# WeltXing/PyDyNet

Hardware: AMD Instinct MI355X
Metric: training-step samples/sec (6L Llama3, seq=256) (higher is better)
Workload: dtype f32

## Files before the change

pydynet_amd/csrc/common.h:

```cpp
#pragma once
#include <hip/hip_runtime.h>
#include <stdint.h>
#include <stdio.h>
#include <string.h>

#define PDN_MAX_DIMS 8

enum {
  PDN_OK = 0,
  PDN_EINVAL = -1,
  PDN_EUNSUPPORTED = -2,
  PDN_EWORKSPACE = -3,
};

void pdn_set_error(const char* fmt, ...);

enum {
  PDN_CNT_ROWRES_CHUNK = 0,
  PDN_CNT_ROWTILE_PLAIN = 1,
  PDN_CNT_ROWTILE_SWIGLU_FWD = 2,
  PDN_CNT_ROWTILE_SWIGLU_BWD = 3,
  PDN_CNT_ROWTILE_ROPE = 4,
  PDN_CNT_ROWTILE_ROWMAX = 5,
  PDN_CNT_ROWRES_CHUNK_EPI = 6,
  PDN_CNT_ATT_P_FWD = 7,
  PDN_CNT_ATT_P_BWD = 8,
  PDN_CNT_ATT_RES_FWD = 9,
  PDN_CNT_ATT_RES_BWD = 10,
  PDN_CNT_ATT_STREAM = 11,
  PDN_CNT_CE_DX_DEFERRED = 12,
  PDN_CNT_CE_DW = 13,
  PDN_CNT_OUTRES = 14,
  PDN_CNT_OUTRES_TN = 15,
  PDN_CNT_LINEAR_RELU_FWD = 16,
  PDN_CNT_LINEAR_DX_MASKED = 17,
  PDN_CNT_CE_SMALL = 18,
  PDN_CNT_TILED_SWIGLU_FWD = 19,
  PDN_CNT_TILED_SWIGLU_BWD = 20,
  PDN_CNT_CONV_QUAD_FWD = 21,
  PDN_CNT_CONV_QUAD_DGRAD = 22,
  PDN_CNT_CONV_QUAD_WGRAD = 23,
  PDN_CNT_PATCH_EMBED_FWD = 24,
  PDN_CNT_PATCH_EMBED_BWD = 25,
  PDN_CNT_L2NORM_FWD = 26,
  PDN_CNT_L2NORM_BWD = 27,
  PDN_CNT_SAMPLE = 28,
  PDN_CNT_DECODE_ROWS = 29,
  PDN_CNT_DECODE_SLOTS = 30,
  PDN_CNT_DECODE_WIDE = 31,
  PDN_CNT_BEAM = 32,
  PDN_CNT_EXTEND = 33,
  PDN_CNT_SPECULATE = 34,
  PDN_CNT_PENALTY = 35,
  PDN_CNT_LOGPROBS = 36,
  PDN_CNT_LMHEAD_SPLIT = 37,
  PDN_CNT_PREFIX = 38,
  PDN_CNT_CE_DX_SPLIT = 39,
  PDN_CNT_CE_DW_SPLIT = 40,
  PDN_CNT_ROWTILE_SPLIT = 41,
  PDN_CNT_OUTRES_TN_SPLIT = 42,
  PDN_CNT_ATT_SEG = 43,
  PDN_CNT_ROW_LOSS = 44,
  PDN_CNT_SMOOTH_LOSS = 45,
  PDN_CNT_SLOTS = 46
};
void pdn_count(int slot);

#define PDN_CHECK_ARG(cond, ...)          \
  do {                                    \
    if (!(cond)) {                        \
      pdn_set_error(__VA_ARGS__);         \
      return PDN_EINVAL;                  \
    }                                     \
  } while (0)

#define PDN_LAUNCH_CHECK()                                            \
  do {                                                                \
    hipError_t _e = hipGetLastError();                                \
    if (_e != hipSuccess) {                                           \
      pdn_set_error("%s:%d launch failed: %s", __FILE__, __LINE__,    \
                    hipGetErrorString(_e));                           \
      return (int)_e;                                                 \
    }                                                                 \
  } while (0)

#define PDN_HIP(call)                                                 \
  do {                                                                \
    hipError_t _e = (call);                                           \
    if (_e != hipSuccess) {                                           \
      pdn_set_error("%s:%d %s: %s", __FILE__, __LINE__, #call,        \
                    hipGetErrorString(_e));                           \
      return (int)_e;                                                 \
    }                                                                 \
  } while (0)

static inline int64_t cdiv64(int64_t a, int64_t b) { return (a + b - 1) / b; }

struct PdnView {
  int ndim;
  int64_t shape[PDN_MAX_DIMS];
  int64_t stride[PDN_MAX_DIMS];
};

__device__ __forceinline__ float wave_sum(float v) {
#pragma unroll
  for (int o = 32; o > 0; o >>= 1) v += __shfl_xor(v, o, 64);
  return v;
}
__device__ __forceinline__ float wave_max(float v) {
#pragma unroll
  for (int o = 32; o > 0; o >>= 1) v = fmaxf(v, __shfl_xor(v, o, 64));
  return v;
}
__device__ __forceinline__ double wave_sum(double v) {
#pragma unroll
  for (int o = 32; o > 0; o >>= 1) v += __shfl_xor(v, o, 64);
  return v;
}

template <typename T>
__device__ __forceinline__ T block_sum(T v, T* smem) {
  v = wave_sum(v);
  const int lane = threadIdx.x & 63, wid = threadIdx.x >> 6, nw = (blockDim.x + 63) >> 6;
  if (nw == 1) return v;
  __syncthreads();
  if (lane == 0) smem[wid] = v;
  __syncthreads();
  T r = (T)0;
  for (int i = 0; i < nw; ++i) r += smem[i];
  return r;
}
__device__ __forceinline__ void lds_barrier() {
  asm volatile("s_waitcnt lgkmcnt(0)" ::: "memory");
  __builtin_amdgcn_s_barrier();
  asm volatile("" ::: "memory");
}
__device__ __forceinline__ float block_sum_lds(float v, float* smem) {
  v = wave_sum(v);
  const int lane = threadIdx.x & 63, wid = threadIdx.x >> 6, nw = (blockDim.x + 63) >> 6;
  if (nw == 1) return v;
  lds_barrier();
  if (lane == 0) smem[wid] = v;
  lds_barrier();
  float r = 0.f;
  for (int i = 0; i < nw; ++i) r += smem[i];
  return r;
}
__device__ __forceinline__ float block_max_lds(float v, float* smem) {
  v = wave_max(v);
  const int lane = threadIdx.x & 63, wid = threadIdx.x >> 6, nw = (blockDim.x + 63) >> 6;
  if (nw == 1) return v;
  lds_barrier();
  if (lane == 0) smem[wid] = v;
  lds_barrier();
  float r = smem[0];
  for (int i = 1; i < nw; ++i) r = fmaxf(r, smem[i]);
  return r;
}
__device__ __forceinline__ float block_max(float v, float* smem) {
  v = wave_max(v);
  const int lane = threadIdx.x & 63, wid = threadIdx.x >> 6, nw = (blockDim.x + 63) >> 6;
  if (nw == 1) return v;
  __syncthreads();
  if (lane == 0) smem[wid] = v;
  __syncthreads();
  float r = smem[0];
  for (int i = 1; i < nw; ++i) r = fmaxf(r, smem[i]);
  return r;
}
```

pydynet_amd/csrc/gemm_outres.hip:

```cpp
#include "common.h"
#include <stdlib.h>

static int pdn_ablation_switch(const char* name) {
  const char* e = getenv(name);
  const int v = e ? atoi(e) : 0;
  if (v) fprintf(stderr, "[pdnhip] WARNING: %s=%d -- timing ablation active, results of the affected kernels are WRONG\n", name, v);
  return v;
}

typedef float f32x16 __attribute__((ext_vector_type(16)));

struct OutResParams {
  const float* A;
  const float* B;
  float* C;
  const float* bias;
  const float* residual;
  int M, K;
  int64_t lda, ldb, ldc;
  const float* lse;
  const int64_t* targets;
  const float* gdev;
  float gscale;
  int kps;
// ... 92 lines not shown
      const int I = min(q * NW + wave, 35);
      *reinterpret_cast<float4*>(smem + buf * PIECE + I * 256 + 4 * lane) = rb[q];
    }
  };

  if (npieces > s0) {
#pragma unroll
    for (int q = 0; q < NQ; ++q) issue_one(0, s0, q);
    if (STAGE) park(0);
  }
  const int arow_i = min(m0 + li, p.M - 1);
  const float* arow = p.A + (int64_t)arow_i * p.lda + 4 * lh;
  float4 a[4];
#pragma unroll
  for (int g = 0; g < 4; ++g) {
    const float4 v = *reinterpret_cast<const float4*>(arow + (int64_t)s0 * OR_KP + 8 * g);
    a[g].x = v.x; a[g].y = v.y; a[g].z = v.z; a[g].w = v.w;
  }
  float ce_lse = 0.f, ce_sc = 0.f;
  int ce_rel = 0;
  if (CE == 1) {
    ce_lse = p.lse[arow_i];
    ce_rel = (int)p.targets[arow_i] - 4 * lh;
    ce_sc = p.gscale * (p.gdev ? p.gdev[0] : 1.f);
  }
  float ce_c2 = 0.f, ce_z = 0.f;
  float ce_m = 0.f;
  if (CE == 2) {
    ce_m = p.lse[arow_i];
    for (int q = 1; q < p.max_parts; ++q) ce_m = fmaxf(ce_m, p.lse[(int64_t)q * p.M + arow_i]);
    ce_c2 = -ce_m * 1.4426950408889634f;
  }

  f32x16 acc[9];
#pragma unroll
  for (int j = 0; j < 9; ++j)
#pragma unroll
    for (int r = 0; r < 16; ++r) acc[j][r] = 0.f;

  const int xl = (li >> 1) & 7;
  const int bnn = (4 * lh) * OR_N + li;
  int bq[4];
#pragma unroll
  for (int g = 0; g < 4; ++g) bq[g] = BT ? li * OR_KP + 4 * ((2 * g + lh) ^ xl) : 0;

  for (int s = s0; s < npieces; ++s) {
    if (STAGE) asm volatile("s_waitcnt lgkmcnt(0)" ::: "memory");
    else if (s == s0) asm volatile("s_waitcnt vmcnt(0)" ::: "memory");
    else asm volatile("s_waitcnt vmcnt(2)" ::: "memory");
    __builtin_amdgcn_s_barrier();
    asm volatile("" ::: "memory");
    const float* Bp = smem + ((s - s0) & 1) * PIECE;
    const int nxt = min(s + 1, npieces - 1);
    const float* anext = arow + (int64_t)nxt * OR_KP;
    float b0[3][4], b1[3][4];
#define OR_LOADB(BX, G, T)                                                                       \
  if (BT) {                                                                                      \
    _Pragma("unroll") for (int j = 0; j < 3; ++j) {                                              \
      const float4 v = *reinterpret_cast<const float4*>(Bp + bq[G] + (3 * (T) + j) * (32 * OR_KP)); \
      BX[j][0] = v.x; BX[j][1] = v.y; BX[j][2] = v.z; BX[j][3] = v.w;                            \
    }                                                                                            \
  } else {                                                                                       \
    _Pragma("unroll") for (int j = 0; j < 3; ++j)                                                \
      _Pragma("unroll") for (int q = 0; q < 4; ++q) BX[j][q] = Bp[bnn + (8 * (G) + q) * OR_N + 32 * (3 * (T) + j)]; \
  }
#define OR_MFMA(BX, AV, T)                                                                       \
  {                                                                                              \
    _Pragma("unroll") for (int j = 0; j < 3; ++j) acc[3 * (T) + j] = __builtin_amdgcn_mfma_f32_32x32x2f32(AV.x, BX[j][0], acc[3 * (T) + j], 0, 0, 0); \
    _Pragma("unroll") for (int j = 0; j < 3; ++j) acc[3 * (T) + j] = __builtin_amdgcn_mfma_f32_32x32x2f32(AV.y, BX[j][1], acc[3 * (T) + j], 0, 0, 0); \
    _Pragma("unroll") for (int j = 0; j < 3; ++j) acc[3 * (T) + j] = __builtin_amdgcn_mfma_f32_32x32x2f32(AV.z, BX[j][2], acc[3 * (T) + j], 0, 0, 0); \
    _Pragma("unroll") for (int j = 0; j < 3; ++j) acc[3 * (T) + j] = __builtin_amdgcn_mfma_f32_32x32x2f32(AV.w, BX[j][3], acc[3 * (T) + j], 0, 0, 0); \
  }
#define OR_STEP(BC, BN, G, T)                                                                    \
  if (3 * (G) + (T) + 1 < 12) { OR_LOADB(BN, (3 * (G) + (T) + 1) / 3, (3 * (G) + (T) + 1) % 3) }  \
  __builtin_amdgcn_sched_barrier(0);                                                             \
  OR_MFMA(BC, av, T)                                                                             \
  __builtin_amdgcn_sched_barrier(0);
    OR_LOADB(b0, 0, 0)
#pragma unroll
    for (int g = 0; g < 4; ++g) {
      float4 av = a[g];
      if (CE == 1) {
        const int c0 = ce_rel - (OR_KP * s + 8 * g);
        av.x = ce_grad(av.x, ce_lse, c0 == 0, ce_sc); av.y = ce_grad(av.y, ce_lse, c0 == 1, ce_sc);
        av.z = ce_grad(av.z, ce_lse, c0 == 2, ce_sc); av.w = ce_grad(av.w, ce_lse, c0 == 3, ce_sc);
      }
      if (CE == 2) {
        const float L2E = 1.4426950408889634f;
        av.x = __builtin_amdgcn_exp2f(fmaf(av.x, L2E, ce_c2)); av.y = __builtin_amdgcn_exp2f(fmaf(av.y, L2E, ce_c2));
        av.z = __builtin_amdgcn_exp2f(fmaf(av.z, L2E, ce_c2)); av.w = __builtin_amdgcn_exp2f(fmaf(av.w, L2E, ce_c2));
        ce_z += (av.x + av.y) + (av.z + av.w);
      }
      if (g < 3 && (!(ABLATE & 2) || s < 1)) {
#pragma unroll
        for (int e = 0; e < 3; ++e)
          if (3 * g + e < NQ) issue_one((s - s0 + 1) & 1, nxt, 3 * g + e);
      }
      __builtin_amdgcn_sched_barrier(0);
      if (g & 1) {
        OR_STEP(b1, b0, g, 0) OR_STEP(b0, b1, g, 1) OR_STEP(b1, b0, g, 2)
      } else {
        OR_STEP(b0, b1, g, 0) OR_STEP(b1, b0, g, 1) OR_STEP(b0, b1, g, 2)
      }
      if (!(ABLATE & 1)) {
        const float4 v = *reinterpret_cast<const float4*>(anext + 8 * g);
        a[g].x = v.x; a[g].y = v.y; a[g].z = v.z; a[g].w = v.w;
      }
      __builtin_amdgcn_sched_barrier(0);
    }
#undef OR_STEP
    if (STAGE) park((s - s0 + 1) & 1);
#undef OR_LOADB
#undef OR_MFMA
  }
  asm volatile("s_waitcnt vmcnt(0)" ::: "memory");

  if (CE == 2 && p.slab) {
    const float z = ce_z + __shfl_xor(ce_z, 32, 64);
    if (lh == 0 && m0 + li < p.M) p.zslab[(int64_t)blockIdx.y * p.M + m0 + li] = z;
  }
  if (CE == 2 && !p.slab) {
    const float z = ce_z + __shfl_xor(ce_z, 32, 64);
    const float izl = 1.f / z;
    const int tgl = min(max((int)p.targets[arow_i], 0), p.K - 1);
    if (lh == 0 && m0 + li < p.M) p.lse_out[m0 + li] = ce_m + __logf(z);
    const int mrem2 = p.M - m0;
    float* __restrict__ Cw = p.C + (int64_t)m0 * p.ldc + li;
    const float* __restrict__ Wc = p.Wt + li;
    const float sc = p.gscale;
#pragma unroll
    for (int r = 0; r < 16; ++r) {
      const int rho = (r & 3) + 8 * (r >> 2) + 4 * lh;
      const float iz = __shfl(izl, rho, 64);
      const int tg = __shfl(tgl, rho, 64);
      if (rho < mrem2) {
#pragma unroll
        for (int j = 0; j < 9; ++j) {
          const float wt = Wc[(unsigned)tg * (unsigned)OR_N + 32 * j];
          Cw[(unsigned)rho * (unsigned)p.ldc + 32 * j] = sc * (acc[j][r] * iz - wt);
        }
      }
    }
    return;
  }
  const bool to_slab = p.slab != nullptr;
  float* __restrict__ Cw = to_slab ? p.slab + ((int64_t)blockIdx.y * p.M + m0) * OR_N : p.C + (int64_t)m0 * p.ldc;
  const float* __restrict__ Rw = (p.residual && !to_slab) ? p.residual + (int64_t)m0 * p.ldc : nullptr;
  const unsigned ldc = to_slab ? (unsigned)OR_N : (unsigned)p.ldc;
  const int mrem = p.M - m0 - 4 * lh;
  const bool full = m0 + 32 <= p.M;
  if (p.ablate_rt & 1) return;
  if (full) {
    float bvs[9];
#pragma unroll
    for (int j = 0; j < 9; ++j) bvs[j] = (p.bias && !to_slab) ? p.bias[32 * j + li] : 0.f;
    const unsigned ldcb = 4u * ldc;
    const unsigned ob0 = (unsigned)(4 * lh) * ldcb + 4u * (unsigned)li;
    float rv[3][16];
    auto load_tile = [&](int j) __attribute__((always_inline)) {
      unsigned o = ob0 + 128u * (unsigned)j;
      asm volatile("" : "+v"(o));
#pragma unroll
      for (int r = 0; r < 16; ++r) {
        rv[j % 3][r] = *reinterpret_cast<const float*>(reinterpret_cast<const char*>(Rw) + o);
        o += ((r & 3) == 3) ? 5u * ldcb : ldcb;
      }
    };
    if (Rw) { load_tile(0); load_tile(1); }
#pragma unroll
    for (int j = 0; j < 9; ++j) {
      if (Rw && j + 2 < 9) load_tile(j + 2);
      __builtin_amdgcn_sched_barrier(0);
      unsigned o = ob0 + 128u * (unsigned)j;
      asm volatile("" : "+v"(o));
#pragma unroll
      for (int r = 0; r < 16; ++r) {
        float v = acc[j][r] + bvs[j];
        if (Rw) v += rv[j % 3][r];
        *reinterpret_cast<float*>(reinterpret_cast<char*>(Cw) + o) = v;
        o += ((r & 3) == 3) ? 5u * ldcb : ldcb;
      }
      __builtin_amdgcn_sched_barrier(0);
    }
    return;
  }
#pragma unroll
  for (int j = 0; j < 9; ++j) {
    const float bv = (p.bias && !to_slab) ? p.bias[32 * j + li] : 0.f;
    unsigned o = (unsigned)(4 * lh) * ldc + li + 32 * j;
    float rv[16];
    if (Rw) {
      unsigned orr = o;
#pragma unroll
      for (int r = 0; r < 16; ++r) {
        rv[r] = (full || (r & 3) + 8 * (r >> 2) < mrem) ? Rw[orr] : 0.f;
        orr += ((r & 3) == 3) ? 5 * ldc : ldc;
      }
    }
#pragma unroll
    for (int r = 0; r < 16; ++r) {
      float v = acc[j][r] + bv;
      if (Rw) v += rv[r];
      if (full || (r & 3) + 8 * (r >> 2) < mrem) Cw[o] = v;
      o += ((r & 3) == 3) ? 5 * ldc : ldc;
    }
  }
}

__global__ __launch_bounds__(256) void outres_splitk_reduce_kernel(const float* __restrict__ slab, int splits, int M,
                                                                    const float* __restrict__ bias,
                                                                    const float* __restrict__ residual,
                                                                    float* __restrict__ C, int64_t ldc) {
  const int64_t i = (int64_t)blockIdx.x * 256 + threadIdx.x;
  if (i >= (int64_t)M * (OR_N / 4)) return;
  const int64_t m = i / (OR_N / 4);
  const int c4 = (int)(i - m * (OR_N / 4));
  float4 acc = *reinterpret_cast<const float4*>(slab + m * OR_N + 4 * c4);
  for (int sp = 1; sp < splits; ++sp) {
    const float4 v = *reinterpret_cast<const float4*>(slab + ((int64_t)sp * M + m) * OR_N + 4 * c4);
    acc.x += v.x; acc.y += v.y; acc.z += v.z; acc.w += v.w;
  }
  if (bias) { const float4 v = *reinterpret_cast<const float4*>(bias + 4 * c4); acc.x += v.x; acc.y += v.y; acc.z += v.z; acc.w += v.w; }
  if (residual) {
    const float4 v = *reinterpret_cast<const float4*>(residual + m * ldc + 4 * c4);
    acc.x += v.x; acc.y += v.y; acc.z += v.z; acc.w += v.w;
  }
  *reinterpret_cast<float4*>(C + m * ldc + 4 * c4) = acc;
}

extern "C" int pdn_gemm_outres_plan(int M, int K, int* nw, int* kps) {
  const int npieces = K / OR_KP, wg8 = (M + 255) / 256, wg4 = (M + 127) / 128;
  *nw = wg8 >= 224 ? 8 : 4;
  *kps = npieces;
  if (wg8 >= 224 || getenv("PDN_OUTRES_NO_SPLIT")) return 1;
  if (!getenv("PDN_OUTRES_NO_PLAN8")) {
    int s8 = (256 + wg8 - 1) / wg8;
    if (s8 > npieces / 24) s8 = npieces / 24;
    if (s8 >= 2 && wg8 * s8 >= 224) {
      *nw = 8;
      *kps = (npieces + s8 - 1) / s8;
      return (npieces + *kps - 1) / *kps;
    }
  }
  if (wg4 >= 224) return 1;
  int splits = (448 + wg4 - 1) / wg4;
  if (splits > npieces / 24) splits = npieces / 24;
  if (splits < 2) return 1;
  *kps = (npieces + splits - 1) / splits;
  return (npieces + *kps - 1) / *kps;
}

static int outres_unsplit_nw(int M) { return (M + 255) / 256 >= 224 ? 8 : 4; }

extern "C" int64_t pdn_gemm_outres_workspace_bytes(int M, int K) {
  int nw, kps;
  const int splits = pdn_gemm_outres_plan(M, K, &nw, &kps);
  return splits > 1 ? (int64_t)splits * M * OR_N * 4 : 0;
}

extern "C" int pdn_gemm_outres_supported(int M, int N, int K, int64_t lda, int64_t ldb, int64_t ldc, int b_trans) {
  return N == OR_N && K >= OR_KP && K % OR_KP == 0 && M >= 1 && lda % 4 == 0 && ldb % 4 == 0 && lda >= K &&
         ldb >= (b_trans ? K : N) && ldc >= N && (int64_t)OR_N * ldb < (1ll << 30) && (int64_t)32 * ldc < (1ll << 30);
}

static int outres_launch(const float* A, const float* B, float* C, const float* bias, const float* residual, int M, int N,
                         int K, int64_t lda, int64_t ldb, int64_t ldc, int b_trans, void* workspace,
                         int64_t workspace_bytes, void* stream, int kb = 0, int64_t b_bstride = 0);

extern "C" int pdn_gemm_outres_f32(const float* A, const float* B, float* C, const float* bias,
                                   const float* residual, int M, int N, int K, int64_t lda, int64_t ldb,
                                   int64_t ldc, int b_trans, void* stream) {
  return outres_launch(A, B, C, bias, residual, M, N, K, lda, ldb, ldc, b_trans, nullptr, 0, stream);
}

extern "C" int pdn_gemm_outres_ws_f32(const float* A, const float* B, float* C, const float* bias,
                                      const float* residual, int M, int N, int K, int64_t lda, int64_t ldb,
                                      int64_t ldc, int b_trans, void* workspace, int64_t workspace_bytes, void* stream) {
  return outres_launch(A, B, C, bias, residual, M, N, K, lda, ldb, ldc, b_trans, workspace, workspace_bytes, stream);
}

int pdn_gemm_prof_begin(int family, double flops, double bytes, void* stream);
void pdn_gemm_prof_end(int token, void* stream);

extern "C" int pdn_gemm_outres_blocks_supported(int M, int kb, int nb) {
  const int K = kb * nb;
  const bool big = (M + 255) / 256 >= 224, mid = (M + 127) / 128 >= 224 && K >= 1536;
  return (kb > 0 && kb % OR_KP == 0 && nb >= 1 && (big || mid)) ? 1 : 0;
}
extern "C" int pdn_gemm_outres_blocks_nt_f32(const float* A, const float* W, int64_t b_block_stride, int kb, int nb, float* C,
                                             const float* residual, int M, int64_t lda, int64_t ldc, void* stream) {
  if (M == 0) return PDN_OK;
  const int K = kb * nb;
  if (!pdn_gemm_outres_blocks_supported(M, kb, nb) || (b_block_stride & 3) || (kb & 3) ||
      !pdn_gemm_outres_supported(M, OR_N, K, lda, K, ldc, 1)) {
    pdn_set_error("pdn_gemm_outres_blocks_nt_f32: unsupported shape M=%d kb=%d nb=%d", M, kb, nb);
    return PDN_EUNSUPPORTED;
  }
  const int tk = pdn_gemm_prof_begin(3, 2.0 * M * (double)OR_N * K, 0.0, stream);
  const int rc = outres_launch(A, W, C, nullptr, residual, M, OR_N, K, lda, kb, ldc, 1, nullptr, 0, stream, kb, b_block_stride);
  pdn_gemm_prof_end(tk, stream);
  return rc;
}

static int outres_launch(const float* A, const float* B, float* C, const float* bias, const float* residual, int M, int N,
                         int K, int64_t lda, int64_t ldb, int64_t ldc, int b_trans, void* workspace,
                         int64_t workspace_bytes, void* stream, int kb, int64_t b_bstride) {
  if (M == 0 || N == 0) return PDN_OK;
  PDN_CHECK_ARG(A && B && C, "pdn_gemm_outres_f32: null operand");
  if (!pdn_gemm_outres_supported(M, N, K, lda, kb > 0 ? K : ldb, ldc, b_trans)) {
    pdn_set_error("pdn_gemm_outres_f32: unsupported shape M=%d N=%d K=%d (N 288, K a multiple of 32, leading "
                  "dimensions multiples of 4)", M, N, K);
    return PDN_EUNSUPPORTED;
  }
  PDN_CHECK_ARG(((((uintptr_t)A | (uintptr_t)B) & 15) == 0), "pdn_gemm_outres_f32: 16-byte alignment required");
  OutResParams p{A, B, C, bias, residual, M, K, lda, ldb, ldc, nullptr, nullptr, nullptr, 0.f, K / OR_KP, nullptr};
  static const int s_pdn_outres_rt_ablate = pdn_ablation_switch("PDN_OUTRES_RT_ABLATE");
  p.ablate_rt = s_pdn_outres_rt_ablate;
  if (kb > 0) {
    p.ppb = kb / OR_KP;
    p.ppb_magic = (unsigned)(((1ull << 32) + (unsigned)p.ppb - 1) / (unsigned)p.ppb);
    p.b_bstride = b_bstride;
  }
  hipStream_t st = (hipStream_t)stream;
  int plan_nw = 8, kps = K / OR_KP;
  int splits = pdn_gemm_outres_plan(M, K, &plan_nw, &kps);
  if (splits > 1 && (!workspace || workspace_bytes < (int64_t)splits * M * OR_N * 4 || (ldc & 3) ||
                     ((uintptr_t)C & 15) || ((uintptr_t)workspace & 15) || ((uintptr_t)bias & 15) || ((uintptr_t)residual & 15))) {
    splits = 1;
    plan_nw = outres_unsplit_nw(M);
  }
  if (splits > 1) { p.kps = kps; p.slab = (float*)workspace; }
  static const int nw_env = getenv("PDN_OUTRES_NW") ? atoi(getenv("PDN_OUTRES_NW")) : 0;
  static const int stage_env = getenv("PDN_OUTRES_STAGE") ? atoi(getenv("PDN_OUTRES_STAGE")) : -1;
  static const int ablate = pdn_ablation_switch("PDN_OUTRES_ABLATE");
  const int nw = nw_env ? nw_env : plan_nw;
  const int stage = stage_env >= 0 ? stage_env : 1;
  const dim3 grid((M + 32 * nw - 1) / (32 * nw), splits);
  pdn_count(PDN_CNT_OUTRES);
#define OR_LAUNCH(BT_, NW_, ST_, AB_) hipLaunchKernelGGL((gemm_outres_kernel<BT_, NW_, ST_, AB_>), grid, dim3(NW_ * 64), 0, st, p)
  if (ablate == 1 && b_trans) OR_LAUNCH(true, 4, 1, 1);
  else if (ablate == 2 && b_trans) OR_LAUNCH(true, 4, 1, 2);
  else if (nw == 8 && b_trans) { if (stage) OR_LAUNCH(true, 8, 1, 0); else OR_LAUNCH(true, 8, 0, 0); }
  else if (nw == 8) { if (stage) OR_LAUNCH(false, 8, 1, 0); else OR_LAUNCH(false, 8, 0, 0); }
  else if (b_trans) { if (stage) OR_LAUNCH(true, 4, 1, 0); else OR_LAUNCH(true, 4, 0, 0); }
  else { if (stage) OR_LAUNCH(false, 4, 1, 0); else OR_LAUNCH(false, 4, 0, 0); }
#undef OR_LAUNCH
  PDN_LAUNCH_CHECK();
  if (splits > 1) {
    const int64_t n4 = (int64_t)M * (OR_N / 4);
    hipLaunchKernelGGL(outres_splitk_reduce_kernel, dim3((unsigned)((n4 + 255) / 256)), dim3(256), 0, st, p.slab, splits, M,
                       bias, residual, C, ldc);
    PDN_LAUNCH_CHECK();
  }
  return PDN_OK;
}

int pdn_outres_ce_dx_launch(const float* logits, int64_t ldl, const float* lse, const int64_t* targets, float gscale,
                            const float* gdev, const float* W, int64_t ldw, float* dx, int64_t ldc,
                            const float* residual, int M, int V, void* workspace, int64_t workspace_bytes, void* stream) {
  OutResParams p{logits, W, dx, nullptr, residual, M, V, ldl, ldw, ldc, lse, targets, gdev, gscale, V / OR_KP, nullptr};
  int nw = 8, kps = V / OR_KP;
  int splits = pdn_gemm_outres_plan(M, V, &nw, &kps);
  if (splits > 1 && (!workspace || workspace_bytes < (int64_t)splits * M * OR_N * 4 || (ldc & 3) || ((uintptr_t)dx & 15) ||
                     ((uintptr_t)workspace & 15) || ((uintptr_t)residual & 15))) {
    splits = 1;
    nw = outres_unsplit_nw(M);
  }
  if (splits > 1) { p.kps = kps; p.slab = (float*)workspace; }
  const dim3 grid((M + 32 * nw - 1) / (32 * nw), splits);
  if (nw == 8) hipLaunchKernelGGL((gemm_outres_kernel<true, 8, 1, 0, 1>), grid, dim3(512), 0, (hipStream_t)stream, p);
  else hipLaunchKernelGGL((gemm_outres_kernel<true, 4, 1, 0, 1>), grid, dim3(256), 0, (hipStream_t)stream, p);
  PDN_LAUNCH_CHECK();
  if (splits > 1) {
    const int64_t n4 = (int64_t)M * (OR_N / 4);
    hipLaunchKernelGGL(outres_splitk_reduce_kernel, dim3((unsigned)((n4 + 255) / 256)), dim3(256), 0, (hipStream_t)stream,
                       p.slab, splits, M, (const float*)nullptr, residual, dx, ldc);
    PDN_LAUNCH_CHECK();
  }
  return PDN_OK;
}

__global__ __launch_bounds__(256) void outres_ce2_reduce_kernel(const float* __restrict__ slab, const float* __restrict__ zslab,
                                                                int splits, int M, const float* __restrict__ rowmax,
                                                                int max_parts, const int64_t* __restrict__ targets,
                                                                const float* __restrict__ W, int64_t ldw, int V, float gscale,
                                                                float* __restrict__ dx, int64_t ldc, float* __restrict__ lse_out) {
  const int64_t i = (int64_t)blockIdx.x * blockDim.x + threadIdx.x;
  if (i >= (int64_t)M * (OR_N / 4)) return;
  const int row = (int)(i / (OR_N / 4)), c4 = (int)(i - (int64_t)row * (OR_N / 4));
  float4 a = *reinterpret_cast<const float4*>(slab + (int64_t)row * OR_N + 4 * c4);
  float z = zslab[row];
  for (int s = 1; s < splits; ++s) {
    const float4 b = *reinterpret_cast<const float4*>(slab + ((int64_t)s * M + row) * OR_N + 4 * c4);
    a.x += b.x; a.y += b.y; a.z += b.z; a.w += b.w;
    z += zslab[(int64_t)s * M + row];
  }
  const int t = min(max((int)targets[row], 0), V - 1);
  const float iz = 1.f / z;
  const float4 wt = *reinterpret_cast<const float4*>(W + (int64_t)t * OR_N + 4 * c4);
  float4 o;
  o.x = gscale * (a.x * iz - wt.x); o.y = gscale * (a.y * iz - wt.y);
  o.z = gscale * (a.z * iz - wt.z); o.w = gscale * (a.w * iz - wt.w);
  *reinterpret_cast<float4*>(dx + (int64_t)row * ldc + 4 * c4) = o;
  if (c4 == 0) {
    float m = rowmax[row];
    for (int q = 1; q < max_parts; ++q) m = fmaxf(m, rowmax[(int64_t)q * M + row]);
    lse_out[row] = m + __logf(z);
  }
}

__global__ __launch_bounds__(256) void outres_wt_transpose_kernel(const float* __restrict__ W, int64_t ldw, int V,
                                                                  float* __restrict__ Wt) {
  __shared__ float tile[32][33];
  const int v0 = blockIdx.x * 32, k0 = blockIdx.y * 32, tx = threadIdx.x & 31, ty = threadIdx.x >> 5;
#pragma unroll
  for (int r = ty; r < 32; r += 8) tile[r][tx] = (v0 + tx < V) ? W[(int64_t)(k0 + r) * ldw + v0 + tx] : 0.f;
  __syncthreads();
#pragma unroll
  for (int r = ty; r < 32; r += 8)
    if (v0 + r < V) Wt[(int64_t)(v0 + r) * OR_N + k0 + tx] = tile[tx][r];
}

int pdn_outres_wt_transpose_launch(const float* W, int64_t ldw, int V, float* Wt, void* stream) {
  hipLaunchKernelGGL(outres_wt_transpose_kernel, dim3((V + 31) / 32, OR_N / 32), dim3(256), 0, (hipStream_t)stream, W, ldw, V, Wt);
  PDN_LAUNCH_CHECK();
  return PDN_OK;
}

extern "C" int pdn_linear_ce_dx_deferred_supported(int64_t M, int V, int K) {
  return (K == OR_N && V % OR_KP == 0 && V >= OR_KP && M >= 1 && M < (1ll << 31) && (int64_t)OR_N * V < (1ll << 30)) ? 1 : 0;
}
extern "C" int64_t pdn_linear_ce_dx_deferred_workspace_bytes(int64_t M, int V, int K) {
  if (!pdn_linear_ce_dx_deferred_supported(M, V, K)) return 0;
  int nw, kps;
  const int splits = pdn_gemm_outres_plan((int)M, V, &nw, &kps);
  return (int64_t)V * OR_N * 4 + (splits > 1 ? (int64_t)splits * M * (OR_N + 1) * 4 : 0);
}
int pdn_outres_ce_dx_deferred_launch(const float* logits, int64_t ldl, const float* rowmax, int max_parts,
                                     const int64_t* targets, float gscale, const float* W, int64_t ldw, float* dx,
                                     int64_t ldc, float* lse_out, int M, int V, void* workspace, int64_t workspace_bytes,
                                     void* stream) {
  OutResParams p{logits, W, dx, nullptr, nullptr, M, V, ldl, ldw, ldc, rowmax, targets, nullptr, gscale, V / OR_KP, nullptr};
  p.lse_out = lse_out;
  p.max_parts = max_parts;
  int nw = 8, kps = V / OR_KP;
  const int splits = pdn_gemm_outres_plan(M, V, &nw, &kps);
  const int64_t wt_floats = (int64_t)V * OR_N;
  PDN_CHECK_ARG(workspace && workspace_bytes >= wt_floats * 4 + (splits > 1 ? (int64_t)splits * M * (OR_N + 1) * 4 : 0) &&
                    (((uintptr_t)workspace | (uintptr_t)dx) & 15) == 0 && (ldc & 3) == 0,
                "pdn_linear_ce_dx_deferred_f32: workspace too small or misaligned");
  float* Wt = (float*)workspace;
  p.Wt = Wt;
  if (splits > 1) {
    p.kps = kps;
    p.slab = Wt + wt_floats;
    p.zslab = p.slab + (int64_t)splits * M * OR_N;
  }
  const dim3 grid((M + 32 * nw - 1) / (32 * nw), splits);
  hipStream_t st = (hipStream_t)stream;
  hipLaunchKernelGGL(outres_wt_transpose_kernel, dim3((V + 31) / 32, OR_N / 32), dim3(256), 0, st, W, ldw, V, Wt);
  PDN_LAUNCH_CHECK();
  pdn_count(PDN_CNT_CE_DX_DEFERRED);
  if (nw == 8) hipLaunchKernelGGL((gemm_outres_kernel<true, 8, 1, 0, 2>), grid, dim3(512), 0, st, p);
  else hipLaunchKernelGGL((gemm_outres_kernel<true, 4, 1, 0, 2>), grid, dim3(256), 0, st, p);
  PDN_LAUNCH_CHECK();
  if (splits > 1) {
    const int64_t n4 = (int64_t)M * (OR_N / 4);
    hipLaunchKernelGGL(outres_ce2_reduce_kernel, dim3((unsigned)((n4 + 255) / 256)), dim3(256), 0, st, p.slab, p.zslab, splits, M,
                       rowmax, max_parts, targets, Wt, ldw, V, gscale, dx, ldc, lse_out);
    PDN_LAUNCH_CHECK();
  }
  return PDN_OK;
}

struct OutResTnParams {
  const float* X;
  const float* G;
  float* C;
  int N, K;
  int64_t ldx, ldg, ldc, slab;
  int k_per_split;
  const float* lse;
  const int64_t* targets;
  const float* gdev;
  float gscale;
  float* colsum;
  int nb_cols;
  int64_t blk_stride;
  int xcd_swizzle;
};

template <int NW, bool CE = false, bool WIDE = false>
__global__ __launch_bounds__(NW * 64, 1) void gemm_outres_tn_kernel(OutResTnParams p) {
  constexpr int PIECE = OR_KP * OR_N;
  constexpr int NQ = (36 + NW - 1) / NW;
  constexpr int GP = OR_KP * 32;
  extern __shared__ __attribute__((aligned(16))) float smem[];
  const int tid = threadIdx.x, lane = tid & 63;
  const int wave = __builtin_amdgcn_readfirstlane(tid >> 6);
  const int li = lane & 31, lh = lane >> 5;
  int bx = blockIdx.x, by = blockIdx.y;
  if (p.xcd_swizzle) {
    const int L = blockIdx.y * gridDim.x + blockIdx.x, xcd = L & 7, slot = L >> 3;
    bx = slot % (int)gridDim.x;
    by = (slot / (int)gridDim.x) * 8 + xcd;
  }
  const int n0_raw = (bx * NW + wave) * 32;
  const bool active = n0_raw < p.N;
  const int n0 = active ? n0_raw : p.N - 32;
  const int k_begin = by * p.k_per_split;
  const int k_end = min(p.K, k_begin + p.k_per_split);
  const int npieces = (k_end - k_begin) / OR_KP;
  const unsigned ldx = (unsigned)p.ldx, ldg = (unsigned)p.ldg;
  const float* Xk = p.X + (int64_t)k_begin * p.ldx;
  float* Gs = smem + 2 * PIECE + wave * (2 * GP);
  float* Ls = smem + 2 * PIECE + NW * 2 * GP;
  const float ce_sc = CE ? p.gscale * (p.gdev ? p.gdev[0] : 1.f) : 0.f;
  float ce_row = 0.f;
  float csum = 0.f;

  float4 rb[NQ], rg[4];
  unsigned xo[NQ];
#pragma unroll
  for (int q = 0; q < NQ; ++q) {
    const int u = 64 * min(q * NW + wave, 35) + lane, k = u / 72, n4 = u - 72 * k;
    xo[q] = (unsigned)k * ldx + 4u * (unsigned)n4;
  }
  auto fetch = [&](int piece, int q) {
    const float4 v = *reinterpret_cast<const float4*>(Xk + (int64_t)piece * OR_KP * p.ldx + xo[q]);
    rb[q].x = v.x; rb[q].y = v.y; rb[q].z = v.z; rb[q].w = v.w;
  };
  const float* gsrc = p.G + (int64_t)(k_begin + (lane >> 3)) * p.ldg + n0 + 4 * (lane & 7);
  auto fetch_g = [&](int piece) {
    const float* g = gsrc + (int64_t)piece * OR_KP * p.ldg;
#pragma unroll
    for (int e = 0; e < 4; ++e) {
      const float4 v = *reinterpret_cast<const float4*>(g + (unsigned)(8 * e) * ldg);
      rg[e].x = v.x; rg[e].y = v.y; rg[e].z = v.z; rg[e].w = v.w;
    }
  };
  auto fetch_rows = [&](int piece) {
    if (CE && wave == 0) {
      const int t = k_begin + piece * OR_KP + li;
      ce_row = lh == 0 ? -1.4426950408889634f * p.lse[t] : __int_as_float((int)p.targets[t]);
    }
  };
  auto park = [&](int buf) {
#pragma unroll
    for (int q = 0; q < NQ; ++q) {
      const int I = min(q * NW + wave, 35);
      *reinterpret_cast<float4*>(smem + buf * PIECE + I * 256 + 4 * lane) = rb[q];
    }
#pragma unroll
    for (int e = 0; e < 4; ++e) *reinterpret_cast<float4*>(Gs + buf * GP + e * 256 + 4 * lane) = rg[e];
    if (CE && wave == 0) Ls[(lh * 2 + buf) * 32 + li] = ce_row;
  };
  if (npieces > 0) {
#pragma unroll
    for (int q = 0; q < NQ; ++q) fetch(0, q);
    fetch_g(0);
    fetch_rows(0);
    park(0);
  }

  f32x16 acc[9];
#pragma unroll
  for (int j = 0; j < 9; ++j)
#pragma unroll
    for (int r = 0; r < 16; ++r) acc[j][r] = 0.f;
  const int bnn = (4 * lh) * OR_N + li;
  const int gnn = (4 * lh) * 32 + li;

  for (int s = 0; s < npieces; ++s) {
    asm volatile("s_waitcnt lgkmcnt(0)" ::: "memory");
    __builtin_amdgcn_s_barrier();
    asm volatile("" ::: "memory");
    const float* Bp = smem + (s & 1) * PIECE;
    const float* Gp = Gs + (s & 1) * GP + gnn;
    const int nxt = min(s + 1, npieces - 1);
    if constexpr (WIDE) {
      const float* Bw = Bp + (4 * lh) * OR_N + 4 * li;
      const float* Bt = Bp + (4 * lh) * OR_N + 256 + li;
      float4 wa[2][2];
      float wt[2];
      auto loadx = [&](int slot, int kk) {
        wa[slot][0] = *reinterpret_cast<const float4*>(Bw + kk * OR_N);
        wa[slot][1] = *reinterpret_cast<const float4*>(Bw + kk * OR_N + 128);
        wt[slot] = Bt[kk * OR_N];
      };
      loadx(0, 0);
      float gn[4];
#pragma unroll
      for (int q = 0; q < 4; ++q) gn[q] = Gp[q * 32];
#pragma unroll
      for (int g = 0; g < 4; ++g) {
        float gv[4];
#pragma unroll
        for (int q = 0; q < 4; ++q) gv[q] = gn[q];
        if (CE) {
          const float4 l4 = *reinterpret_cast<const float4*>(Ls + (s & 1) * 32 + 8 * g + 4 * lh);
          const float4 t4 = *reinterpret_cast<const float4*>(Ls + (2 + (s & 1)) * 32 + 8 * g + 4 * lh);
          const int col = n0 + li;
          gv[0] = ce_unscaled(gv[0], l4.x, __float_as_int(t4.x) == col);
          gv[1] = ce_unscaled(gv[1], l4.y, __float_as_int(t4.y) == col);
          gv[2] = ce_unscaled(gv[2], l4.z, __float_as_int(t4.z) == col);
          gv[3] = ce_unscaled(gv[3], l4.w, __float_as_int(t4.w) == col);
          csum += (gv[0] + gv[1]) + (gv[2] + gv[3]);
        }
        if (g + 1 < 4) {
#pragma unroll
          for (int q = 0; q < 4; ++q) gn[q] = Gp[(8 * (g + 1) + q) * 32];
        }
        if (g == 0) { fetch_g(nxt); fetch_rows(nxt); }
        if (g < 3) {
#pragma unroll
          for (int e = 0; e < 3; ++e)
            if (3 * g + e < NQ) fetch(nxt, 3 * g + e);
        }
        __builtin_amdgcn_sched_barrier(0);
#pragma unroll
        for (int q = 0; q < 4; ++q) {
          const int cur = q & 1;
          if (4 * g + q + 1 < 16) loadx(cur ^ 1, 8 * ((4 * g + q + 1) >> 2) + ((4 * g + q + 1) & 3));
          __builtin_amdgcn_sched_barrier(0);
          acc[0] = __builtin_amdgcn_mfma_f32_32x32x2f32(wa[cur][0].x, gv[q], acc[0], 0, 0, 0);
          acc[1] = __builtin_amdgcn_mfma_f32_32x32x2f32(wa[cur][0].y, gv[q], acc[1], 0, 0, 0);
          acc[2] = __builtin_amdgcn_mfma_f32_32x32x2f32(wa[cur][0].z, gv[q], acc[2], 0, 0, 0);
          acc[3] = __builtin_amdgcn_mfma_f32_32x32x2f32(wa[cur][0].w, gv[q], acc[3], 0, 0, 0);
          acc[4] = __builtin_amdgcn_mfma_f32_32x32x2f32(wa[cur][1].x, gv[q], acc[4], 0, 0, 0);
          acc[5] = __builtin_amdgcn_mfma_f32_32x32x2f32(wa[cur][1].y, gv[q], acc[5], 0, 0, 0);
          acc[6] = __builtin_amdgcn_mfma_f32_32x32x2f32(wa[cur][1].z, gv[q], acc[6], 0, 0, 0);
          acc[7] = __builtin_amdgcn_mfma_f32_32x32x2f32(wa[cur][1].w, gv[q], acc[7], 0, 0, 0);
          acc[8] = __builtin_amdgcn_mfma_f32_32x32x2f32(wt[cur], gv[q], acc[8], 0, 0, 0);
          __builtin_amdgcn_sched_barrier(0);
// ... 156 lines not shown
```

Baseline: 7757.

## Route output-resident N=288 GEMMs through split-fp16 MFMA kernel with streamed activations

Adds a new path for the output-resident GEMM (N=288) that splits fp32 operands into high/low fp16 pairs with per-column and per-row power-of-two scaling. It then runs three 16x16x32 f16 MFMAs per tile in place of the fp32 MFMA kernel. Weights are first converted to a split fp16 image by two prep kernels. A persistent main kernel streams activation rows through an LDS ring and rescales accumulators when the exponent changes. The aim is to gain fp16 matrix-core throughput while keeping near-fp32 accuracy, at the cost of extra prep launches, a temporary allocation per call, and possible precision differences.

```diff
diff --git a/pydynet_amd/csrc/common.h b/pydynet_amd/csrc/common.h
--- a/pydynet_amd/csrc/common.h
+++ b/pydynet_amd/csrc/common.h
@@ -62,7 +62,8 @@
   PDN_CNT_ATT_SEG = 43,
   PDN_CNT_ROW_LOSS = 44,
   PDN_CNT_SMOOTH_LOSS = 45,
-  PDN_CNT_SLOTS = 46
+  PDN_CNT_OUTRES_SPLIT = 46,
+  PDN_CNT_SLOTS = 47
 };
 void pdn_count(int slot);
 
diff --git a/pydynet_amd/csrc/gemm_outres.hip b/pydynet_amd/csrc/gemm_outres.hip
--- a/pydynet_amd/csrc/gemm_outres.hip
+++ b/pydynet_amd/csrc/gemm_outres.hip
@@ -418,6 +418,12 @@
   return rc;
 }
 
+int pdn_outres_split_takes(const float* A, const float* B, const float* C, const float* bias, const float* residual, int M,
+                           int K, int64_t lda, int64_t ldb, int64_t ldc, int b_trans, int kb, int64_t b_bstride, int splits,
+                           void* stream);
+int pdn_outres_split_launch(const float* A, const float* B, float* C, const float* bias, const float* residual, int M, int K,
+                            int64_t lda, int64_t ldb, int64_t ldc, int b_trans, int kb, int64_t b_bstride, void* stream);
+
 static int outres_launch(const float* A, const float* B, float* C, const float* bias, const float* residual, int M, int N,
                          int K, int64_t lda, int64_t ldb, int64_t ldc, int b_trans, void* workspace,
                          int64_t workspace_bytes, void* stream, int kb, int64_t b_bstride) {
@@ -446,6 +452,11 @@
     plan_nw = outres_unsplit_nw(M);
   }
   if (splits > 1) { p.kps = kps; p.slab = (float*)workspace; }
+  if (pdn_outres_split_takes(A, B, C, bias, residual, M, K, lda, ldb, ldc, b_trans, kb, b_bstride, splits, stream)) {
+    const int rc = pdn_outres_split_launch(A, B, C, bias, residual, M, K, lda, ldb, ldc, b_trans, kb, b_bstride, stream);
+    if (rc == PDN_OK) pdn_count(PDN_CNT_OUTRES);
+    return rc;
+  }
   static const int nw_env = getenv("PDN_OUTRES_NW") ? atoi(getenv("PDN_OUTRES_NW")) : 0;
   static const int stage_env = getenv("PDN_OUTRES_STAGE") ? atoi(getenv("PDN_OUTRES_STAGE")) : -1;
   static const int ablate = pdn_ablation_switch("PDN_OUTRES_ABLATE");
diff --git a/pydynet_amd/csrc/outres_split.hip b/pydynet_amd/csrc/outres_split.hip
--- /dev/null
+++ b/pydynet_amd/csrc/outres_split.hip
@@ -0,0 +1,366 @@
+#include "split_tn.h"
+#include "outres_split_index.h"
+
+extern "C" int pdn_malloc(void** ptr, int64_t bytes);
+extern "C" int pdn_free(void* ptr);
+
+struct OrsWParams {
+  const float* B;
+  float* pmax;
+  int* wsh;
+  char* wimg;
+  int np, ppb;
+  int64_t ldb, bstride;
+};
+
+__device__ __forceinline__ float ors_finite_or_inf(float a) { return a < INFINITY ? a : INFINITY; }
+
+template <bool NN>
+__device__ __forceinline__ void ors_w_unit(const OrsWParams& p, const float* tile, int d, int q, float (&v)[8]) {
+  if (NN) {
+#pragma unroll
+    for (int j = 0; j < 8; ++j) v[j] = tile[ors_nn_lds(8 * q + j, d)];
+  } else {
+    const float* src = p.B + ors_w_src_nt(blockIdx.x, d, q, p.ppb, p.ldb, p.bstride);
+    const float4 a = *reinterpret_cast<const float4*>(src);
+    const float4 b = *reinterpret_cast<const float4*>(src + 4);
+    v[0] = a.x; v[1] = a.y; v[2] = a.z; v[3] = a.w; v[4] = b.x; v[5] = b.y; v[6] = b.z; v[7] = b.w;
+  }
+}
+__device__ __forceinline__ void ors_w_stage_nn(const OrsWParams& p, float* tile) {
+  for (int i = threadIdx.x; i < ORS_KP * (ORS_N / 4); i += 256) {
+    const float4 a = *reinterpret_cast<const float4*>(p.B + ors_w_src_nn(blockIdx.x, i, p.ldb));
+    float* t = tile + ors_nn_lds(i / 72, 4 * (i % 72));
+    t[0] = a.x; t[1] = a.y; t[2] = a.z; t[3] = a.w;
+  }
+  __syncthreads();
+}
+
+template <bool NN>
+__global__ __launch_bounds__(256) void ors_w_max_kernel(OrsWParams p) {
+  __shared__ float tile[NN ? ORS_KP * ORS_NN_LD : 1];
+  if (NN) ors_w_stage_nn(p, tile);
+  for (int i = threadIdx.x; i < ORS_N * 4; i += 256) {
+    const int d = i >> 2, q = i & 3;
+    float v[8];
+    ors_w_unit<NN>(p, tile, d, q, v);
+    float m = 0.f;
+#pragma unroll
+    for (int j = 0; j < 8; ++j) m = fmaxf(m, ors_finite_or_inf(fabsf(v[j])));
+    m = fmaxf(m, __shfl_xor(m, 1, 64));
+    m = fmaxf(m, __shfl_xor(m, 2, 64));
+    if (q == 0) p.pmax[(int64_t)blockIdx.x * ORS_N + d] = m;
+  }
+}
+
+template <bool NN>
+__global__ __launch_bounds__(256) void ors_w_img_kernel(OrsWParams p) {
+  __shared__ float tile[NN ? ORS_KP * ORS_NN_LD : 1];
+  if (NN) ors_w_stage_nn(p, tile);
+  char* img = p.wimg + (int64_t)blockIdx.x * ORS_PIECE;
+  for (int i = threadIdx.x; i < ORS_N * 4; i += 256) {
+    const int d = i >> 2, q = i & 3;
+    float amax = 0.f;
+    for (int s = 0; s < p.np; ++s) amax = fmaxf(amax, p.pmax[(int64_t)s * ORS_N + d]);
+    const int sh = ls_shift(amax);
+    if (blockIdx.x == 0 && q == 0) p.wsh[d] = sh;
+    float v[8];
+    ors_w_unit<NN>(p, tile, d, q, v);
+    f16x8 hv, lv;
+#pragma unroll
+    for (int j = 0; j < 8; ++j) {
+      _Float16 h, l;
+      ls_split(v[j], sh, h, l);
+      hv[j] = h; lv[j] = l;
+    }
+    char* dst = img + ors_img_unit(d, q);
+    *reinterpret_cast<f16x8*>(dst) = hv;
+    *reinterpret_cast<f16x8*>(dst + ORS_PLANE) = lv;
+  }
+}
+
+struct OrsParams {
+  const float* A;
+  const char* wimg;
+  const int* wsh;
+  const float* bias;
+  const float* residual;
+  float* C;
+  int M, np, nblk;
+  int64_t lda, ldc;
+};
+
+__device__ __forceinline__ float ors_max8(const float4& a, const float4& b) {
+  const float v[8] = {a.x, a.y, a.z, a.w, b.x, b.y, b.z, b.w};
+  float m = 0.f;
+#pragma unroll
+  for (int j = 0; j < 8; ++j) {
+    const float f = fabsf(v[j]);
+    m = fmaxf(m, f < INFINITY ? f : 0.f);
+  }
+  return m;
+}
+__device__ __forceinline__ int ors_step_exp(float mx, int S) { return ors_next_exp(mx > 0.f, __builtin_amdgcn_frexp_expf(mx), S); }
+__device__ __forceinline__ void ors_form2(float x0, float x1, int S, unsigned& hp, unsigned& lp) {
+  f16x2 h, l;
+  _Float16 a, b;
+  ls_split_scaled(ldexpf(x0, S), a, b);
+  h[0] = a; l[0] = b;
+  ls_split_scaled(ldexpf(x1, S), a, b);
+  h[1] = a; l[1] = b;
+  hp = __builtin_bit_cast(unsigned, h);
+  lp = __builtin_bit_cast(unsigned, l);
+  asm volatile("" : "+v"(hp), "+v"(lp));
+}
+
+template <int ABLATE>
+__global__ __launch_bounds__(512, 1) void ors_main_kernel(OrsParams p) {
+  __shared__ __attribute__((aligned(1024))) char smem[ORS_LDS];
+  const int tid = threadIdx.x, lane = tid & 63;
+  const int wave = __builtin_amdgcn_readfirstlane(tid >> 6);
+  const int r = lane & 15, q = lane >> 4;
+  const int np = p.np, nblk = p.nblk, grid = gridDim.x;
+  const unsigned lds0 = (unsigned)(size_t)(__attribute__((address_space(3))) char*)smem;
+  constexpr bool STREAM = ABLATE == 0 || ABLATE == 3;
+
+  const char* wsrc = p.wimg + lane * 16;
+  auto dma_w = [&](int piece, int slot) __attribute__((always_inline)) {
+    const char* src = wsrc + (int64_t)piece * ORS_PIECE;
+#pragma unroll
+    for (int e = 0; e < 5; ++e) {
+      const int I = ors_wdma_instr(e, wave);
+      split_dma16(src + I * 1024, __builtin_amdgcn_readfirstlane(lds0 + slot + I * 1024));
+    }
+  };
+  auto a_src = [&](int blk, int i) __attribute__((always_inline)) {
+    return p.A + ors_a_row(blk, wave, ors_raw_row(i, lane), p.M) * p.lda + 4 * ors_raw_chunk(i, lane);
+  };
+  int blk = blockIdx.x, nxt = ors_next_block(blk, grid, nblk);
+  const float* ac0 = a_src(blk, 0);
+  const float* ac1 = a_src(blk, 1);
+  const float* an0 = a_src(nxt, 0);
+  const float* an1 = a_src(nxt, 1);
+  const int rw_base = ORS_RING0 + wave * (ORS_RING * ORS_RAW);
+  auto dma_raw = [&](const float* s0, const float* s1, int piece, int ring) __attribute__((always_inline)) {
+    const int64_t o = (int64_t)piece * ORS_KP;
+    split_dma16(s0 + o, __builtin_amdgcn_readfirstlane(lds0 + rw_base + ring * ORS_RAW));
+    split_dma16(s1 + o, __builtin_amdgcn_readfirstlane(lds0 + rw_base + ring * ORS_RAW + 1024));
+  };
+  const int raw_lane = rw_base + ors_raw_lane(r, q);
+
+  dma_w(0, 0);
+  if (ABLATE != 1) { dma_raw(ac0, ac1, 0, 0); dma_raw(ac0, ac1, 1, 1); dma_raw(ac0, ac1, 2, 2); dma_raw(ac0, ac1, 3, 3); }
+  asm volatile("s_waitcnt vmcnt(0)" ::: "memory");
+  f16x8 bh, bl;
+#pragma unroll
+  for (int j = 0; j < 8; ++j) { bh[j] = (_Float16)1.f; bl[j] = (_Float16)0.5f; }
+  int S = ABLATE == 1 ? 0 : ORS_UNSET;
+  if (ABLATE != 1) {
+    const float4 v0 = *reinterpret_cast<const float4*>(__builtin_assume_aligned(smem + raw_lane, 16));
+    const float4 v1 = *reinterpret_cast<const float4*>(__builtin_assume_aligned(smem + (raw_lane ^ 16), 16));
+    float mx = ors_max8(v0, v1);
+    mx = fmaxf(mx, __shfl_xor(mx, 16, 64));
+    mx = fmaxf(mx, __shfl_xor(mx, 32, 64));
+    S = ors_step_exp(mx, S);
+    unsigned h0, h1, h2, h3, l0, l1, l2, l3;
+    ors_form2(v0.x, v0.y, S, h0, l0);
+    ors_form2(v0.z, v0.w, S, h1, l1);
+    ors_form2(v1.x, v1.y, S, h2, l2);
+    ors_form2(v1.z, v1.w, S, h3, l3);
+    bh = stn_pack4(h0, h1, h2, h3); bl = stn_pack4(l0, l1, l2, l3);
+  }
+
+  f32x4 acc0[ORS_NT], acc1[ORS_NT];
+#pragma unroll
+  for (int j = 0; j < ORS_NT; ++j)
+#pragma unroll
+    for (int i = 0; i < 4; ++i) { acc0[j][i] = 0.f; acc1[j][i] = 0.f; }
+
+  const int frag = ors_frag(r, q);
+  constexpr int TOPWAIT = STREAM ? 2 : 0;
+
+  int cur = 0, g = 0;
+  for (;;) {
+    int Snext = ORS_UNSET;
+    for (int s = 0; s < np; ++s, ++g) {
+      asm volatile("s_waitcnt vmcnt(%0)" ::"n"(TOPWAIT) : "memory");
+      __builtin_amdgcn_s_barrier();
+      asm volatile("" ::: "memory");
+      const char* fb = smem + cur + frag;
+      const bool last = s + 1 == np;
+      f16x8 wh[2], wl[2];
+      u32x4 nh = __builtin_bit_cast(u32x4, bh), nl = __builtin_bit_cast(u32x4, bl);
+      float4 rv0 = make_float4(0.f, 0.f, 0.f, 0.f), rv1 = rv0;
+      float mx = 0.f, mo = 0.f;
+      int Sn = last ? ORS_UNSET : S;
+#define ORS_LOADW(X, J)                                                                                  \
+  {                                                                                                      \
+    wh[X] = *reinterpret_cast<const f16x8*>(__builtin_assume_aligned(fb + (J) * 1024, 16));              \
+    wl[X] = *reinterpret_cast<const f16x8*>(__builtin_assume_aligned(fb + (J) * 1024 + ORS_PLANE, 16));  \
+  }
+      ORS_LOADW(0, 0)
+#pragma unroll
+      for (int j = 0; j < ORS_NT; ++j) {
+        if (j + 1 < ORS_NT) { ORS_LOADW((j + 1) & 1, j + 1) }
+        if (j == 0) {
+          dma_w(last ? 0 : s + 1, ORS_PIECE - cur);
+          if (STREAM) {
+            const bool ahead = ors_ahead_next(s, np);
+            dma_raw(ahead ? an0 : ac0, ahead ? an1 : ac1, ors_ahead_piece(s, np), g & (ORS_RING - 1));
+          }
+          if (ABLATE != 1) {
+            const int ro = raw_lane + ((g + 1) & (ORS_RING - 1)) * ORS_RAW;
+            rv0 = *reinterpret_cast<const float4*>(__builtin_assume_aligned(smem + ro, 16));
+            rv1 = *reinterpret_cast<const float4*>(__builtin_assume_aligned(smem + (ro ^ 16), 16));
+          }
+        }
+        __builtin_amdgcn_sched_barrier(0);
+        acc0[j] = __builtin_amdgcn_mfma_f32_16x16x32_f16(wh[j & 1], bh, acc0[j], 0, 0, 0);
+        acc1[j] = __builtin_amdgcn_mfma_f32_16x16x32_f16(wl[j & 1], bh, acc1[j], 0, 0, 0);
+        acc1[j] = __builtin_amdgcn_mfma_f32_16x16x32_f16(wh[j & 1], bl, acc1[j], 0, 0, 0);
+        if (ABLATE != 1) {
+          if (j == 1) { mx = ors_max8(rv0, rv1); mo = __shfl_xor(mx, 16, 64); }
+          if (j == 2) { mx = fmaxf(mx, mo); mo = __shfl_xor(mx, 32, 64); }
+          if (j == 3) { mx = fmaxf(mx, mo); Sn = ors_step_exp(mx, Sn); }
+          if (j >= 5 && (j - 5) % 3 == 0 && j <= 14) {
+            const int e = (j - 5) / 3;
+            const float4 rv = (e >> 1) ? rv1 : rv0;
+            unsigned hp, lp;
+            ors_form2((e & 1) ? rv.z : rv.x, (e & 1) ? rv.w : rv.y, Sn, hp, lp);
+            if (e == 0) { nh.x = hp; nl.x = lp; } else if (e == 1) { nh.y = hp; nl.y = lp; }
+            else if (e == 2) { nh.z = hp; nl.z = lp; } else { nh.w = hp; nl.w = lp; }
+            __builtin_amdgcn_sched_group_barrier(0x008, 1, 0);
+            __builtin_amdgcn_sched_group_barrier(0x002, 6, 0);
+            __builtin_amdgcn_sched_group_barrier(0x008, 1, 0);
+            __builtin_amdgcn_sched_group_barrier(0x002, 6, 0);
+            __builtin_amdgcn_sched_group_barrier(0x008, 1, 0);
+          }
+        }
+        __builtin_amdgcn_sched_barrier(0);
+      }
+#undef ORS_LOADW
+      bh = __builtin_bit_cast(f16x8, nh); bl = __builtin_bit_cast(f16x8, nl);
+      cur = ORS_PIECE - cur;
+      if (last) {
+        Snext = Sn;
+      } else {
+        if (__builtin_amdgcn_ballot_w64(Sn != S) != 0) {
+          const float f = ldexpf(1.f, Sn - S);
+#pragma unroll
+          for (int j = 0; j < ORS_NT; ++j) { acc0[j] *= f; acc1[j] *= f; }
+        }
+        S = Sn;
+      }
+    }
+
+    const int64_t row = (int64_t)blk * ORS_WG_ROWS + wave * 16 + r;
+    if ((ABLATE != 3 || p.M < 0) && row < p.M) {
+      float* out = p.C + row * p.ldc + 4 * q;
+      const float* res = p.residual ? p.residual + row * p.ldc + 4 * q : nullptr;
+      const float* bia = p.bias ? p.bias + 4 * q : nullptr;
+      const int* __restrict__ shp = p.wsh + 4 * q;
+#pragma unroll
+      for (int j = 0; j < ORS_NT; ++j) {
+        const int4 sv = *reinterpret_cast<const int4*>(shp + 16 * j);
+        float4 o;
+        o.x = stn_unscale(acc1[j][0], acc0[j][0], S + sv.x);
+        o.y = stn_unscale(acc1[j][1], acc0[j][1], S + sv.y);
+        o.z = stn_unscale(acc1[j][2], acc0[j][2], S + sv.z);
+        o.w = stn_unscale(acc1[j][3], acc0[j][3], S + sv.w);
+        if (bia) { const float4 b4 = *reinterpret_cast<const float4*>(bia + 16 * j); o.x += b4.x; o.y += b4.y; o.z += b4.z; o.w += b4.w; }
+        if (res) { const float4 r4 = *reinterpret_cast<const float4*>(res + 16 * j); o.x += r4.x; o.y += r4.y; o.z += r4.z; o.w += r4.w; }
+        *reinterpret_cast<float4*>(out + 16 * j) = o;
+      }
+    }
+    asm volatile("s_waitcnt vmcnt(0)" ::: "memory");
+    if (nxt == blk) break;
+    blk = nxt;
+    nxt = ors_next_block(blk, grid, nblk);
+    ac0 = an0; ac1 = an1;
+    an0 = a_src(nxt, 0); an1 = a_src(nxt, 1);
+    S = ABLATE == 1 ? 0 : Snext;
+#pragma unroll
+    for (int j = 0; j < ORS_NT; ++j)
+#pragma unroll
+      for (int i = 0; i < 4; ++i) { acc0[j][i] = 0.f; acc1[j][i] = 0.f; }
+  }
+}
+
+namespace {
+struct OrsTemp {
+  void* p = nullptr;
+  hipStream_t st = nullptr;
+  int get(int64_t bytes, void* stream) { st = (hipStream_t)stream; return pdn_malloc(&p, bytes); }
+  ~OrsTemp() {
+    static const bool two_stream = getenv("PDN_TWO_STREAM") && atoi(getenv("PDN_TWO_STREAM")) != 0;
+    if (p && two_stream) (void)hipStreamSynchronize(st);
+    if (p) pdn_free(p);
+  }
+};
+}
+
+int pdn_outres_split_takes(const float* A, const float* B, const float* C, const float* bias, const float* residual, int M,
+                           int K, int64_t lda, int64_t ldb, int64_t ldc, int b_trans, int kb, int64_t b_bstride, int splits,
+                           void* stream) {
+  if (M < ORS_MIN_ROWS || K < ORS_MIN_K || K > ORS_MAX_K || K % ORS_KP != 0 || splits != 1) return 0;
+  if ((lda & 3) || (ldc & 3) || (ldb & 3) || (b_bstride & 3) || lda < K || ldc < ORS_N) return 0;
+  if (kb > 0 ? (!b_trans || kb % ORS_KP != 0 || K % kb != 0) : ldb < (b_trans ? K : ORS_N)) return 0;
+  if (((uintptr_t)A | (uintptr_t)B | (uintptr_t)C | (uintptr_t)bias | (uintptr_t)residual) & 15) return 0;
+  const char* e = getenv("PDN_OUTRES_SPLIT");
+  if (e && atoi(e) == 0) {
+    static bool s_told = false;
+    if (!s_told) {
+      s_told = true;
+      fprintf(stderr, "[pdnhip] WARNING: PDN_OUTRES_SPLIT=0 -- the layer input gradients and the down projection stay on the fp32 MFMA kernel\n");
+    }
+    return 0;
+  }
+  hipStreamCaptureStatus cs = hipStreamCaptureStatusNone;
+  if (hipStreamIsCapturing((hipStream_t)stream, &cs) != hipSuccess) { (void)hipGetLastError(); return 0; }
+  return cs == hipStreamCaptureStatusNone ? 1 : 0;
+}
+
+int pdn_outres_split_launch(const float* A, const float* B, float* C, const float* bias, const float* residual, int M, int K,
+                            int64_t lda, int64_t ldb, int64_t ldc, int b_trans, int kb, int64_t b_bstride, void* stream) {
+  const char* ea = getenv("PDN_OUTRES_SPLIT_ABLATE");
+  const int ablate = ea ? atoi(ea) : 0;
+  if (ablate != 0) {
+    static bool s_told = false;
+    if (!s_told) {
+      s_told = true;
+      fprintf(stderr, "[pdnhip] WARNING: PDN_OUTRES_SPLIT_ABLATE=%d -- timing ablation active, the results of the split output-resident products are WRONG\n", ablate);
+    }
+  }
+  const char* eg = getenv("PDN_OUTRES_SPLIT_WGS");
+  const int env_wgs = eg ? atoi(eg) : -1;
+  const int np = K / ORS_KP;
+  OrsTemp tmp;
+  const int rc = tmp.get((int64_t)np * ORS_PIECE + (int64_t)np * ORS_N * 4 + ORS_N * 4, stream);
+  if (rc) return rc;
+  hipStream_t st = (hipStream_t)stream;
+  OrsWParams w;
+  memset(&w, 0, sizeof(w));
+  w.B = B; w.wimg = static_cast<char*>(tmp.p); w.pmax = reinterpret_cast<float*>(w.wimg + (int64_t)np * ORS_PIECE);
+  w.wsh = reinterpret_cast<int*>(w.pmax + (int64_t)np * ORS_N);
+  w.np = np; w.ppb = kb > 0 ? kb / ORS_KP : np; w.ldb = ldb; w.bstride = kb > 0 ? b_bstride : 0;
+  if (b_trans) {
+    hipLaunchKernelGGL(ors_w_max_kernel<false>, dim3(np), dim3(256), 0, st, w);
+    hipLaunchKernelGGL(ors_w_img_kernel<false>, dim3(np), dim3(256), 0, st, w);
+  } else {
+    hipLaunchKernelGGL(ors_w_max_kernel<true>, dim3(np), dim3(256), 0, st, w);
+    hipLaunchKernelGGL(ors_w_img_kernel<true>, dim3(np), dim3(256), 0, st, w);
+  }
+  OrsParams p;
+  memset(&p, 0, sizeof(p));
+  p.A = A; p.wimg = w.wimg; p.wsh = w.wsh; p.bias = bias; p.residual = residual; p.C = C;
+  p.M = M; p.np = np; p.nblk = ors_blocks(M); p.lda = lda; p.ldc = ldc;
+  int wgs = ors_grid(M);
+  if (env_wgs == 0) wgs = p.nblk;
+  else if (env_wgs > 0) wgs = ors_min_i(env_wgs, p.nblk);
+  const dim3 grid((unsigned)wgs);
+  if (ablate == 3) hipLaunchKernelGGL(ors_main_kernel<3>, grid, dim3(512), 0, st, p);
+  else STN_LAUNCH_ABLATE(ors_main_kernel, ablate, grid, stream, p);
+  pdn_count(PDN_CNT_OUTRES_SPLIT);
+  PDN_LAUNCH_CHECK();
+  return PDN_OK;
+}
diff --git a/pydynet_amd/csrc/outres_split_index.h b/pydynet_amd/csrc/outres_split_index.h
--- /dev/null
+++ b/pydynet_amd/csrc/outres_split_index.h
@@ -0,0 +1,53 @@
+#pragma once
+#include <stdint.h>
+
+#if defined(__HIPCC__) || defined(__CUDACC__)
+#define ORS_HD __host__ __device__ __forceinline__
+#else
+#define ORS_HD inline
+#endif
+
+#define ORS_N 288
+#define ORS_NT 18
+#define ORS_KP 32
+#define ORS_PLANE (ORS_N * ORS_KP * 2)
+#define ORS_PIECE (2 * ORS_PLANE)
+#define ORS_RAW 2048
+#define ORS_RING 4
+#define ORS_WG_ROWS 128
+#define ORS_RING0 (2 * ORS_PIECE)
+#define ORS_LDS (ORS_RING0 + 8 * ORS_RING * ORS_RAW)
+#define ORS_MAX_WGS 256
+#define ORS_MIN_ROWS 65536
+#define ORS_MIN_K 256
+#define ORS_MAX_K 4096
+#define ORS_NN_LD 289
+
+ORS_HD int ors_min_i(int a, int b) { return a < b ? a : b; }
+ORS_HD int64_t ors_min_l(int64_t a, int64_t b) { return a < b ? a : b; }
+
+ORS_HD int ors_blocks(int64_t M) { return (int)((M + ORS_WG_ROWS - 1) / ORS_WG_ROWS); }
+ORS_HD int ors_grid(int64_t M) { return ors_min_i(ors_blocks(M), ORS_MAX_WGS); }
+ORS_HD int ors_next_block(int blk, int grid, int nblk) { return blk + grid < nblk ? blk + grid : blk; }
+
+ORS_HD int ors_img_unit(int d, int q) { return (d * 4 + (q ^ ((d >> 2) & 3))) * 16; }
+ORS_HD int ors_frag(int r, int q) { return ors_img_unit(r, q); }
+ORS_HD int64_t ors_w_src_nt(int piece, int d, int q, int ppb, int64_t ldb, int64_t bstride) {
+  const int b = piece / ppb;
+  return (int64_t)b * bstride + (int64_t)d * ldb + (int64_t)(piece - b * ppb) * ORS_KP + 8 * q;
+}
+ORS_HD int64_t ors_w_src_nn(int piece, int i, int64_t ldb) { return ((int64_t)piece * ORS_KP + i / 72) * ldb + 4 * (i % 72); }
+ORS_HD int ors_nn_lds(int k, int d) { return k * ORS_NN_LD + d; }
+ORS_HD int ors_wdma_instr(int e, int wave) { return ors_min_i(e * 8 + wave, 35); }
+
+ORS_HD int ors_raw_row(int i, int lane) { return 8 * i + (lane >> 3); }
+ORS_HD int ors_raw_chunk(int i, int lane) { return (lane & 7) ^ ((ors_raw_row(i, lane) >> 1) & 7); }
+ORS_HD int64_t ors_a_row(int blk, int wave, int rr, int64_t M) { return ors_min_l((int64_t)blk * ORS_WG_ROWS + wave * 16 + rr, M - 1); }
+ORS_HD int ors_raw_lane(int r, int q) { return r * 128 + (((2 * q) ^ ((r >> 1) & 7)) << 4); }
+ORS_HD int ors_ahead_piece(int s, int np) { return s + ORS_RING < np ? s + ORS_RING : s + ORS_RING - np; }
+ORS_HD bool ors_ahead_next(int s, int np) { return s + ORS_RING >= np; }
+
+ORS_HD int ors_out_col(int j, int q) { return 16 * j + 4 * q; }
+
+#define ORS_UNSET (1 << 20)
+ORS_HD int ors_next_exp(bool nonzero, int E, int S) { return (nonzero && E + S >= 16) ? 13 - E : S; }
```

Result: faster. 8443, median of 6 (+8.8%).
